# summmeer/session-based-news-recommendation

Measured on AMD Instinct MI355X. Metric: sessions/sec TCAR train on Globo (synthetic globo fold), higher is better.
Workload: dtype bf16 (logits GEMM on split-bf16 planes = 3 MFMAs per product, gradient GEMMs plain bf16; fp32 accumulate, fp32 master state)

## Files before the change

session-based-news-recommendation_amd/csrc/gemm_f32.hip:

```cpp
#include "tcar_common.h"
#include "tcar_bf16_layout.h"
#include <stdlib.h>

typedef __attribute__((ext_vector_type(16))) float f32x16;

constexpr int BK = 32;
constexpr int MAXP = 10;
constexpr int MAXSEG = 3;

struct GemmProb {
  const float* A[MAXSEG];
  const float* B[MAXSEG];
  long lda[MAXSEG], ldb[MAXSEG];
  int K[MAXSEG];
  int nseg;
  float* C;
  long ldc;
  const float* bias;
  int M, N, act, beta;
  int ksplit, kchunk, mode;
  int mt, nt, wg_begin;
  int dact; const float* dact_y; long ld_dact_y; float* colsum;
  __bf16* plane_hi; __bf16* plane_lo; int plane_in32, plane_col0;
  __bf16* pack_hi; __bf16* pack_lo; int pack_in32, pack_c0, pack_c1;
};
struct GroupArgs {
  int nprob;
  int wg0[MAXP];
  GemmProb p[MAXP];
  TcarSignal sig;
};

template <int LAY, int ROWS>
struct TileGeo {
  static constexpr int KC_LD = BK + 4;
  static constexpr int MC_LD = ROWS + 4;
  static constexpr int FLOATS = (LAY == 0) ? ROWS * KC_LD : BK * MC_LD;
  static constexpr int NV = ROWS * BK / 4 / 256;
};

template <int LAY, int ROWS>
__device__ __forceinline__ void load_tile(const float* __restrict__ P, long ld, int r0, int rmax, int k0, int kend,
                                          int tid, float4 (&reg)[TileGeo<LAY, ROWS>::NV]) {
#pragma unroll
  for (int i = 0; i < TileGeo<LAY, ROWS>::NV; ++i) {
    const int f = tid + 256 * i;
    if (LAY == 0) {
      const int row = f >> 3, c4 = f & 7;
      const int gr = r0 + row, gk = k0 + c4 * 4;
      reg[i] = (gr < rmax && gk < kend) ? ld4(P + (long)gr * ld + gk) : zero4();
    } else {
      constexpr int C4 = ROWS / 4;
      const int krow = f / C4, c4 = f - krow * C4;
      const int gk = k0 + krow, gr = r0 + c4 * 4;
      reg[i] = (gk < kend && gr + 3 < rmax) ? ld4(P + (long)gk * ld + gr) : zero4();
    }
  }
}
template <int LAY, int ROWS>
__device__ __forceinline__ void store_tile(float* __restrict__ S, int tid, const float4 (&reg)[TileGeo<LAY, ROWS>::NV]) {
#pragma unroll
  for (int i = 0; i < TileGeo<LAY, ROWS>::NV; ++i) {
    const int f = tid + 256 * i;
    if (LAY == 0) {
      const int row = f >> 3, c4 = f & 7;
      st4(S + row * TileGeo<LAY, ROWS>::KC_LD + c4 * 4, reg[i]);
    } else {
      constexpr int C4 = ROWS / 4;
      const int krow = f / C4, c4 = f - krow * C4;
      st4(S + krow * TileGeo<LAY, ROWS>::MC_LD + c4 * 4, reg[i]);
    }
  }
}
template <int LAY, int ROWS>
__device__ __forceinline__ void read_frag(const float* __restrict__ S, int idx, int c, int h, float (&out)[4]) {
  if (LAY == 0) {
    const float4 v = ld4(S + idx * TileGeo<LAY, ROWS>::KC_LD + c * 8 + 4 * h);
    out[0] = v.x; out[1] = v.y; out[2] = v.z; out[3] = v.w;
  } else {
#pragma unroll
    for (int j = 0; j < 4; ++j) out[j] = S[(c * 8 + 4 * h + j) * TileGeo<LAY, ROWS>::MC_LD + idx];
  }
}

template <int LA, int LB, int TM, int TN>
__global__ __launch_bounds__(256, 2) void gemm_f32_kernel(const GroupArgs ga) {
  extern __shared__ __attribute__((aligned(16))) float smem[];
  constexpr int FM = TM / 64, FN = TN / 64;
  constexpr int A_FL = TileGeo<LA, TM>::FLOATS, B_FL = TileGeo<LB, TN>::FLOATS;
  constexpr int STAGE = A_FL + B_FL;
  const int tid = threadIdx.x;
  const int wave = tid >> 6, lane = tid & 63;
  const int wm = wave >> 1, wn = wave & 1;
  const int li = lane & 31, lh = lane >> 5;

  const int nwg = gridDim.x, bid = blockIdx.x;
  const int xcd = bid & 7, q = nwg >> 3, r = nwg & 7;
  int id = (xcd < r ? xcd * (q + 1) : r * (q + 1) + (xcd - r) * q) + (bid >> 3);
  int pi = 0;
#pragma unroll
  for (int i = 1; i < MAXP; ++i) pi += (id >= ga.wg0[i]) ? 1 : 0;
  const GemmProb& g = ga.p[pi];
  id -= g.wg_begin;
  const int tiles = g.mt * g.nt;
  const int split = id / tiles;
  id -= split * tiles;
  int tm, tn;
  if (g.mt <= g.nt) { tn = id / g.mt; tm = id - tn * g.mt; } else { tm = id / g.nt; tn = id - tm * g.nt; }
  const int m0 = tm * TM, n0 = tn * TN;

  f32x16 acc[FM][FN];
#pragma unroll
  for (int a = 0; a < FM; ++a)
#pragma unroll
    for (int b = 0; b < FN; ++b)
#pragma unroll
      for (int e = 0; e < 16; ++e) acc[a][b][e] = 0.f;

  float4 ra[TileGeo<LA, TM>::NV], rb[TileGeo<LB, TN>::NV];
#pragma unroll 1
  for (int sg = 0; sg < g.nseg; ++sg) {
    const float* __restrict__ Ap = g.A[sg];
    const float* __restrict__ Bp = g.B[sg];
    const long lda = g.lda[sg], ldb = g.ldb[sg];
    const int Kseg = g.K[sg];
    const int ks = split * g.kchunk;
    const int ke = min(Kseg, ks + g.kchunk);
    const int nit = (ke - ks + BK - 1) / BK;
    const int a_rmax = (LA == 0) ? g.M : min((int)lda, (g.M + 3) & ~3);
    const int b_rmax = (LB == 0) ? g.N : min((int)ldb, (g.N + 3) & ~3);
    if (nit > 0) {
      load_tile<LA, TM>(Ap, lda, m0, a_rmax, ks, ke, tid, ra);
      load_tile<LB, TN>(Bp, ldb, n0, b_rmax, ks, ke, tid, rb);
      __syncthreads();
      store_tile<LA, TM>(smem, tid, ra);
      store_tile<LB, TN>(smem + A_FL, tid, rb);
    }
    __syncthreads();
    for (int it = 0; it < nit; ++it) {
      const float* As = smem + (it & 1) * STAGE;
      const float* Bs = As + A_FL;
      const bool more = (it + 1 < nit);
      if (more) {
        load_tile<LA, TM>(Ap, lda, m0, a_rmax, ks + (it + 1) * BK, ke, tid, ra);
        load_tile<LB, TN>(Bp, ldb, n0, b_rmax, ks + (it + 1) * BK, ke, tid, rb);
      }
#pragma unroll
      for (int c = 0; c < BK / 8; ++c) {
        float a[FM][4], b[FN][4];
#pragma unroll
        for (int s = 0; s < FM; ++s) read_frag<LA, TM>(As, wm * (TM / 2) + s * 32 + li, c, lh, a[s]);
#pragma unroll
        for (int s = 0; s < FN; ++s) read_frag<LB, TN>(Bs, wn * (TN / 2) + s * 32 + li, c, lh, b[s]);
#pragma unroll
        for (int j = 0; j < 4; ++j)
#pragma unroll
          for (int s = 0; s < FM; ++s)
#pragma unroll
            for (int t = 0; t < FN; ++t)
              acc[s][t] = __builtin_amdgcn_mfma_f32_32x32x2f32(a[s][j], b[t][j], acc[s][t], 0, 0, 0);
      }
      if (more) {
        float* An = smem + ((it + 1) & 1) * STAGE;
        store_tile<LA, TM>(An, tid, ra);
        store_tile<LB, TN>(An + A_FL, tid, rb);
      }
      __syncthreads();
    }
  }

  float* Cs = g.C + (g.mode == 1 ? (long)split * g.M * g.ldc : 0L);
#pragma unroll
  for (int s = 0; s < FM; ++s)
#pragma unroll
    for (int t = 0; t < FN; ++t) {
      const int col = n0 + wn * (TN / 2) + t * 32 + li;
      if (col >= g.N) continue;
      const float bv = g.bias ? g.bias[col] : 0.f;
#pragma unroll
      for (int e = 0; e < 16; ++e) {
        const int row = m0 + wm * (TM / 2) + s * 32 + (e & 3) + 8 * (e >> 2) + 4 * lh;
        if (row < g.M) {
          float* p = Cs + (long)row * g.ldc + col;
          if (g.mode == 2) {
            atomicAdd(p, acc[s][t][e]);
          } else {
            float v = acc[s][t][e] + bv;
            if (g.act == 1) v = fmaxf(v, 0.f);
            else if (g.act == 2) v = tanhf(v);
            if (g.beta) v += *p;
            *p = v;
          }
        }
      }
    }
}

__global__ __launch_bounds__(256) void splitk_reduce_kernel(const float* __restrict__ slabs, int splitk, int M, int N,
                                                             long ld, float* __restrict__ out) {
  const long n4 = N >> 2;
  const long total = (long)M * n4;
  for (long i = (long)blockIdx.x * blockDim.x + threadIdx.x; i < total; i += (long)gridDim.x * blockDim.x) {
    const long row = i / n4, c = (i - row * n4) * 4;
    float4 s = zero4();
    for (int k = 0; k < splitk; ++k) s = add4(s, ld4(slabs + ((long)k * M + row) * ld + c));
    st4(out + row * ld + c, s);
  }
}

typedef __attribute__((ext_vector_type(8))) __bf16 xbf16x8;
typedef __attribute__((ext_vector_type(4))) __bf16 xbf16x4;
constexpr int X3_MC = 192;
template <int XK> struct X3 {
  static constexpr int KC = 2 * XK + 16;
  static constexpr int PLANE = XK * X3_MC;
  static constexpr int NV = 64 * XK / 4 / 256;
};

typedef float v4f __attribute__((ext_vector_type(4)));
__device__ __forceinline__ v4f gload16_hidden(const float* p) {
  v4f v;
  asm volatile("global_load_dwordx4 %0, %1, off" : "=v"(v) : "v"(p) : "memory");
  return v;
}
template <int N, int NV>
__device__ __forceinline__ void x3_wait(v4f (&a)[NV], v4f (&b)[NV]) {
  static_assert(NV == 2 || NV == 4 || NV == 8, "stage depth 32 / 64 / 128");
  if constexpr (NV == 2)
    asm volatile("s_waitcnt vmcnt(%4)" : "+v"(a[0]), "+v"(a[1]), "+v"(b[0]), "+v"(b[1]) : "n"(N) : "memory");
  else if constexpr (NV == 4)
    asm volatile("s_waitcnt vmcnt(%8)"
                 : "+v"(a[0]), "+v"(a[1]), "+v"(a[2]), "+v"(a[3]), "+v"(b[0]), "+v"(b[1]), "+v"(b[2]), "+v"(b[3])
                 : "n"(N) : "memory");
  else
    asm volatile("s_waitcnt vmcnt(%16)"
                 : "+v"(a[0]), "+v"(a[1]), "+v"(a[2]), "+v"(a[3]), "+v"(a[4]), "+v"(a[5]), "+v"(a[6]), "+v"(a[7]), "+v"(b[0]),
                   "+v"(b[1]), "+v"(b[2]), "+v"(b[3]), "+v"(b[4]), "+v"(b[5]), "+v"(b[6]), "+v"(b[7])
                 : "n"(N) : "memory");
}

template <int LAY, int XK>
__device__ __forceinline__ unsigned x3_load(const float* __restrict__ P, long ld, int r0, int rmax, int k0, int kend, int tid,
                                            v4f (&reg)[X3<XK>::NV]) {
  unsigned mask = 0;
#pragma unroll
  for (int i = 0; i < X3<XK>::NV; ++i) {
    const int f = tid + 256 * i;
    bool ok;
    long off;
    if (LAY == 0) {
      const int row = f / (XK / 4), c4 = f % (XK / 4);
      const int gr = r0 + row, gk = k0 + c4 * 4;
      ok = gr < rmax && gk < kend;
      off = (long)gr * ld + gk;
    } else {
      const int krow = f >> 4, c4 = f & 15;
      const int gk = k0 + krow, gr = r0 + c4 * 4;
      ok = gk < kend && gr + 3 < rmax;
      off = (long)gk * ld + gr;
    }
    reg[i] = gload16_hidden(P + (ok ? off : 0L));
    mask |= ok ? (1u << i) : 0u;
  }
  return mask;
}
template <int LAY, int XK, bool HI = false>
__device__ __forceinline__ void x3_store(char* __restrict__ hi, char* __restrict__ lo, int tid, const v4f (&reg)[X3<XK>::NV],
                                         unsigned mask) {
#pragma unroll
  for (int i = 0; i < X3<XK>::NV; ++i) {
    const int f = tid + 256 * i;
    const bool ok = (mask >> i) & 1u;
    const float v[4] = {ok ? reg[i].x : 0.f, ok ? reg[i].y : 0.f, ok ? reg[i].z : 0.f, ok ? reg[i].w : 0.f};
    xbf16x4 h, l;
#pragma unroll
    for (int j = 0; j < 4; ++j) { h[j] = (__bf16)v[j]; l[j] = HI ? (__bf16)0.f : (__bf16)(v[j] - (float)h[j]); }
    int off;
    if (LAY == 0) { const int row = f / (XK / 4), c4 = f % (XK / 4); off = row * X3<XK>::KC + c4 * 8; }
    else { const int krow = f >> 4, c4 = f & 15; off = krow * X3_MC + c4 * 8; }
    *reinterpret_cast<xbf16x4*>(hi + off) = h;
    if (!HI) *reinterpret_cast<xbf16x4*>(lo + off) = l;
  }
}
template <int LAY, int XK>
__device__ __forceinline__ xbf16x8 x3_frag(const char* __restrict__ S, int base, int s, int lane) {
  if (LAY == 0) {
    return *reinterpret_cast<const xbf16x8*>(S + (base + (lane & 31)) * X3<XK>::KC + s * 32 + (lane >> 5) * 16);
  } else {
    const int g = lane >> 4, i = lane & 15;
    const int mbase = 16 * (g & 1), kbase = 8 * (g >> 1), q = i >> 2, p = i & 3;
    const char* a0 = S + (s * 16 + kbase + q) * X3_MC + (base + mbase + 4 * p) * 2;
    typedef __attribute__((address_space(3))) xbf16x4* lds_p;
    const xbf16x4 lo = __builtin_amdgcn_ds_read_tr16_b64_v4bf16((lds_p)(a0));
    const xbf16x4 hi = __builtin_amdgcn_ds_read_tr16_b64_v4bf16((lds_p)(a0 + 4 * X3_MC));
    return __builtin_shufflevector(lo, hi, 0, 1, 2, 3, 4, 5, 6, 7);
  }
}

template <int LA, int LB, int XK, int XD, bool HI = false>
__global__ __launch_bounds__(256) void gemm_x3_kernel(const GroupArgs ga) {
  constexpr int X3_PLANE = X3<XK>::PLANE, X3_NV = X3<XK>::NV;
  extern __shared__ __attribute__((aligned(16))) float smem_f[];
  char* smem = reinterpret_cast<char*>(smem_f);
  constexpr int T = 64;
  const int tid = threadIdx.x, wave = tid >> 6, lane = tid & 63;
  const int wm = wave >> 1, wn = wave & 1;
  const int nwg = gridDim.x, bid = blockIdx.x;
  const int xcd = bid & 7, q = nwg >> 3, r = nwg & 7;
  int id = (xcd < r ? xcd * (q + 1) : r * (q + 1) + (xcd - r) * q) + (bid >> 3);
  int pi = 0;
#pragma unroll
  for (int i = 1; i < MAXP; ++i) pi += (id >= ga.wg0[i]) ? 1 : 0;
  const GemmProb& g = ga.p[pi];
  id -= g.wg_begin;
  const int tiles = g.mt * g.nt;
  const int split = id / tiles;
  id -= split * tiles;
  int tm, tn;
  if (g.mt <= g.nt) { tn = id / g.mt; tm = id - tn * g.mt; } else { tm = id / g.nt; tn = id - tm * g.nt; }
  const int m0 = tm * T, n0 = tn * T;

  const int ks = split * g.kchunk;
  int cst[MAXSEG + 1];
  cst[0] = 0;
#pragma unroll
  for (int sg = 0; sg < MAXSEG; ++sg) {
    int n = 0;
    if (sg < g.nseg) {
      const int ke = min(g.K[sg], ks + g.kchunk);
      n = ke > ks ? (ke - ks + XK - 1) / XK : 0;
    }
    cst[sg + 1] = cst[sg] + n;
  }
  const int total = cst[MAXSEG];
  const int a_rmax0 = (LA == 0) ? g.M : (g.M + 3) & ~3;
  const int b_rmax0 = (LB == 0) ? g.N : (g.N + 3) & ~3;

  auto stage_seg = [&](int s) { return min((s >= cst[1] ? 1 : 0) + (s >= cst[2] ? 1 : 0), g.nseg - 1); };
  auto load_stage = [&](int s, v4f (&ra)[X3_NV], v4f (&rb)[X3_NV], unsigned& ma, unsigned& mb) {
    const int sg = stage_seg(s);
    const int k0 = ks + (s - cst[sg]) * XK;
    const int ke = min(g.K[sg], ks + g.kchunk);
    const long lda = g.lda[sg], ldb = g.ldb[sg];
    const int a_rmax = (LA == 0) ? a_rmax0 : min((int)lda, a_rmax0);
    const int b_rmax = (LB == 0) ? b_rmax0 : min((int)ldb, b_rmax0);
    ma = x3_load<LA, XK>(g.A[sg], lda, m0, a_rmax, k0, ke, tid, ra);
    mb = x3_load<LB, XK>(g.B[sg], ldb, n0, b_rmax, k0, ke, tid, rb);
  };

  f32x16 acc;
#pragma unroll
  for (int e = 0; e < 16; ++e) acc[e] = 0.f;
  v4f ra[XD][X3_NV], rb[XD][X3_NV];
  unsigned ma[XD], mb[XD];
#pragma unroll
  for (int d = 0; d < XD; ++d) load_stage(d, ra[d], rb[d], ma[d], mb[d]);
#pragma unroll 1
  for (int base = 0; base < total; base += XD) {
#pragma unroll
    for (int d = 0; d < XD; ++d) {
      const int s = base + d;
      __syncthreads();
      x3_wait<(XD - 1) * 2 * X3_NV, X3_NV>(ra[d], rb[d]);
      x3_store<LA, XK, HI>(smem, smem + X3_PLANE, tid, ra[d], ma[d]);
      x3_store<LB, XK, HI>(smem + 2 * X3_PLANE, smem + 3 * X3_PLANE, tid, rb[d], mb[d]);
      __syncthreads();
      load_stage(s + XD, ra[d], rb[d], ma[d], mb[d]);
      const int sg = stage_seg(s);
      const int k0 = ks + (s - cst[sg]) * XK;
      const int left = min(g.K[sg], ks + g.kchunk) - k0;
      const int nsub = s < total ? (min(XK, left + 15) >> 4) : 0;
#pragma unroll 2
      for (int u = 0; u < nsub; ++u) {
        const xbf16x8 ah = x3_frag<LA, XK>(smem, wm * 32, u, lane), bh = x3_frag<LB, XK>(smem + 2 * X3_PLANE, wn * 32, u, lane);
        if constexpr (!HI) {
          const xbf16x8 al = x3_frag<LA, XK>(smem + X3_PLANE, wm * 32, u, lane), bl = x3_frag<LB, XK>(smem + 3 * X3_PLANE, wn * 32, u, lane);
          acc = __builtin_amdgcn_mfma_f32_32x32x16_bf16(al, bh, acc, 0, 0, 0);
          acc = __builtin_amdgcn_mfma_f32_32x32x16_bf16(ah, bl, acc, 0, 0, 0);
        }
        acc = __builtin_amdgcn_mfma_f32_32x32x16_bf16(ah, bh, acc, 0, 0, 0);
      }
    }
  }
  asm volatile("s_waitcnt vmcnt(0)" ::: "memory");
  float* Cs = g.C + (g.mode == 1 ? (long)split * g.M * g.ldc : 0L);
  const bool wt = ga.sig.cnt != nullptr;
  const int col = n0 + wn * 32 + (lane & 31);
  float csum = 0.f;
  if (col < g.N) {
    const float bv = g.bias ? g.bias[col] : 0.f;
    const int gcol = g.plane_col0 + col;
    const bool packed = g.pack_hi && (gcol < g.pack_c0 || gcol >= g.pack_c1);
    const int pcol = gcol < g.pack_c0 ? gcol : gcol - (g.pack_c1 - g.pack_c0);
#pragma unroll
    for (int e = 0; e < 16; ++e) {
      const int row = m0 + wm * 32 + (e & 3) + 8 * (e >> 2) + 4 * (lane >> 5);
      if (row < g.M) {
        float* p = Cs + (long)row * g.ldc + col;
        if (g.mode == 2) {
          atomicAdd(p, acc[e]);
        } else {
          float v = acc[e] + bv;
          if (g.act == 1) v = fmaxf(v, 0.f);
          else if (g.act == 2) v = tanhf(v);
          if (g.dact) {
            const float y = g.dact_y[(long)row * g.ld_dact_y + col];
            v = g.dact == 1 ? (y > 0.f ? v : 0.f) : v * (1.f - y * y);
            csum += v;
          }
          if (g.beta) v += *p;
          if (wt) __hip_atomic_store(p, v, __ATOMIC_RELAXED, __HIP_MEMORY_SCOPE_AGENT);
          else *p = v;
          if (g.plane_hi) {
            const __bf16 h = (__bf16)v, l = (__bf16)(v - (float)h);
            const long o = kb32_off(row, gcol, g.plane_in32);
            g.plane_hi[o] = h;
            g.plane_lo[o] = l;
            if (packed) {
              const long po = kb32_off(row, pcol, g.pack_in32);
              g.pack_hi[po] = h;
              g.pack_lo[po] = l;
            }
          }
        }
      }
    }
  }
  if (g.dact && g.colsum) {
    csum += __shfl_xor(csum, 32);
    if (lane < 32 && col < g.N && csum != 0.f) atomicAdd(g.colsum + col, csum);
  }
  tcar_signal_done(ga.sig);
}

namespace {

template <int LA, int LB, int TM, int TN>
int launch_variant(const GroupArgs& ga, int nwg, hipStream_t st) {
  constexpr size_t lds = 2 * (TileGeo<LA, TM>::FLOATS + TileGeo<LB, TN>::FLOATS) * sizeof(float);
  TCAR_SET_LDS_ONCE((gemm_f32_kernel<LA, LB, TM, TN>), lds);
  TCAR_LAUNCH((gemm_f32_kernel<LA, LB, TM, TN>), dim3(nwg), dim3(256), lds, st, ga);
  TCAR_CHECK_LAUNCH();
  return TCAR_OK;
}

template <int LA, int LB>
int launch_layout(GroupArgs& ga, hipStream_t st) {
  long big = 0;
  for (int i = 0; i < ga.nprob; ++i)
    big += (long)((ga.p[i].M + 127) / 128) * ((ga.p[i].N + 127) / 128) * ga.p[i].ksplit;
  const int T = big >= 192 ? 128 : 64;
  int wg = 0;
  for (int i = 0; i < ga.nprob; ++i) {
    GemmProb& p = ga.p[i];
    p.mt = (p.M + T - 1) / T;
    p.nt = (p.N + T - 1) / T;
    p.wg_begin = wg;
    ga.wg0[i] = wg;
    wg += p.mt * p.nt * p.ksplit;
  }
  for (int i = ga.nprob; i < MAXP; ++i) ga.wg0[i] = 0x7fffffff;
  if (T == 128) return launch_variant<LA, LB, 128, 128>(ga, wg, st);
  return launch_variant<LA, LB, 64, 64>(ga, wg, st);
}

template <int LA, int LB, int XK, int XD, bool HI = false>
int launch_x3_v(GroupArgs& ga, int wg, hipStream_t st, TcarOpt* o) {
  constexpr size_t lds = 4 * X3<XK>::PLANE;
  if (o && o->sig.cnt)
    for (int i = 0; i < ga.nprob; ++i)
      if (ga.p[i].plane_hi || ga.p[i].pack_hi) return TCAR_E_ARG;
  ga.sig = tcar_sig(o);
  TCAR_SET_LDS_ONCE((gemm_x3_kernel<LA, LB, XK, XD, HI>), lds);
  TCAR_LAUNCH((gemm_x3_kernel<LA, LB, XK, XD, HI>), dim3(wg), dim3(256), lds, st, ga);
  TCAR_CHECK_LAUNCH();
  return TCAR_OK;
}

template <int LA, int LB>
int launch_x3(GroupArgs& ga, hipStream_t st, TcarOpt* o) {
  int wg = 0;
  for (int i = 0; i < ga.nprob; ++i) {
    GemmProb& p = ga.p[i];
    p.mt = (p.M + 63) / 64;
    p.nt = (p.N + 63) / 64;
    p.wg_begin = wg;
    ga.wg0[i] = wg;
    wg += p.mt * p.nt * p.ksplit;
  }
  for (int i = ga.nprob; i < MAXP; ++i) ga.wg0[i] = 0x7fffffff;
  int max_stages = 0;
  for (int i = 0; i < ga.nprob; ++i) {
    const GemmProb& p = ga.p[i];
    int n = 0;
    for (int sg = 0; sg < p.nseg; ++sg) n += ((p.K[sg] < p.kchunk ? p.K[sg] : p.kchunk) + 63) / 64;
    max_stages = n > max_stages ? n : max_stages;
  }
  if constexpr (LA == LB)
    if (o && o->hi_only)
      return max_stages <= tcar_fixed::x3_oneshot ? launch_x3_v<LA, LB, 64, 2, true>(ga, wg, st, o) : launch_x3_v<LA, LB, 64, 1, true>(ga, wg, st, o);
  if (max_stages <= tcar_fixed::x3_oneshot) return launch_x3_v<LA, LB, 64, 2>(ga, wg, st, o);
  if constexpr (tcar_fixed::x3_deep != 0)
    if (wg <= 256) return launch_x3_v<LA, LB, 128, 1>(ga, wg, st, o);
  return launch_x3_v<LA, LB, 64, 1>(ga, wg, st, o);
}

int fill_prob(GemmProb& p, int layout, const tcar_gemm_desc_t& d) {
  if (d.M <= 0 || d.N <= 0 || d.nseg < 1 || d.nseg > MAXSEG || !d.C) return TCAR_E_ARG;
  const bool a_kc = (layout != 2), b_kc = (layout == 1);
  p.nseg = d.nseg;
  for (int s = 0; s < d.nseg; ++s) {
    if (!d.A[s] || !d.B[s] || d.K[s] <= 0 || !tcar_aligned16(d.A[s]) || !tcar_aligned16(d.B[s]) || (d.lda[s] & 3) ||
        (d.ldb[s] & 3))
      return TCAR_E_ARG;
    if ((a_kc || b_kc) && (d.K[s] & 3)) return TCAR_E_ARG;
    p.A[s] = d.A[s]; p.B[s] = d.B[s]; p.lda[s] = d.lda[s]; p.ldb[s] = d.ldb[s]; p.K[s] = d.K[s];
  }
  p.C = d.C; p.ldc = d.ldc; p.bias = d.bias; p.M = d.M; p.N = d.N; p.act = d.act; p.beta = d.beta;
  p.dact = d.dact; p.dact_y = d.dact_y; p.ld_dact_y = d.ld_dact_y; p.colsum = d.colsum;
  if (d.dact && (d.dact < 1 || d.dact > 2 || !d.dact_y)) return TCAR_E_ARG;
  p.plane_hi = (__bf16*)d.plane_hi; p.plane_lo = (__bf16*)d.plane_lo; p.plane_in32 = d.plane_inner >> 5; p.plane_col0 = d.plane_col0;
  p.pack_hi = (__bf16*)d.pack_hi; p.pack_lo = (__bf16*)d.pack_lo; p.pack_in32 = d.pack_inner >> 5;
  p.pack_c0 = d.pack_c0; p.pack_c1 = d.pack_c1;
  if (d.plane_hi && (!d.plane_lo || (d.plane_inner & 31) || d.plane_col0 < 0 || d.plane_col0 + d.N > d.plane_inner)) return TCAR_E_ARG;
  if (d.pack_hi && (!d.plane_hi || !d.pack_lo || (d.pack_inner & 31) || d.pack_c0 > d.pack_c1)) return TCAR_E_ARG;
  if ((d.dact || d.plane_hi) && d.splitk > 1) return TCAR_E_ARG;
  int splitk = d.splitk < 1 ? 1 : d.splitk;
  p.mode = splitk > 1 ? (d.atomic ? 2 : 1) : 0;
  if (splitk > 1 && (d.nseg != 1 || d.bias || d.act || d.beta)) return TCAR_E_ARG;
  int kmax = 0;
  for (int s = 0; s < d.nseg; ++s) kmax = d.K[s] > kmax ? d.K[s] : kmax;
  int kchunk = (kmax + splitk - 1) / splitk;
  kchunk = ((kchunk + BK - 1) / BK) * BK;
  p.kchunk = kchunk;
  p.ksplit = (kmax + kchunk - 1) / kchunk;
  if (p.ksplit == 1) p.mode = (splitk > 1 && d.atomic) ? 2 : 0;
  return TCAR_OK;
}

}

extern "C" int tcar_gemm_f32_grouped(int layout, int nprob, const tcar_gemm_desc_t* descs, void* stream) {
  if (nprob <= 0) return TCAR_OK;
  if (layout < 0 || layout > 2 || nprob > MAXP || !descs) return TCAR_E_ARG;
  GroupArgs ga;
  ga.nprob = 0;
  for (int i = 0; i < nprob; ++i) {
    if (descs[i].M <= 0 || descs[i].N <= 0) continue;
    const int rc = fill_prob(ga.p[ga.nprob], layout, descs[i]);
    if (rc) return rc;
    ga.nprob++;
  }
  if (ga.nprob == 0) return TCAR_OK;
  hipStream_t st = (hipStream_t)stream;
  if (layout == 0) return launch_layout<0, 1>(ga, st);
  if (layout == 1) return launch_layout<0, 0>(ga, st);
  return launch_layout<1, 1>(ga, st);
}

extern "C" int tcar_gemm_x3_grouped(int layout, int nprob, const tcar_gemm_desc_t* descs, void* stream) {
  return tcar_gemm_x3_grouped_o(layout, nprob, descs, stream, nullptr);
}
int tcar_gemm_x3_grouped_o(int layout, int nprob, const tcar_gemm_desc_t* descs, void* stream, TcarOpt* o) {
  if (nprob <= 0) return TCAR_OK;
  if (layout < 0 || layout > 2 || nprob > MAXP || !descs) return TCAR_E_ARG;
  GroupArgs ga;
  ga.nprob = 0;
  for (int i = 0; i < nprob; ++i) {
    if (descs[i].M <= 0 || descs[i].N <= 0) continue;
    const int rc = fill_prob(ga.p[ga.nprob], layout, descs[i]);
    if (rc) return rc;
    ga.nprob++;
  }
  if (ga.nprob == 0) return TCAR_OK;
  hipStream_t st = (hipStream_t)stream;
  if (layout == 0) return launch_x3<0, 1>(ga, st, o);
  if (layout == 1) return launch_x3<0, 0>(ga, st, o);
  return launch_x3<1, 1>(ga, st, o);
}

extern "C" int tcar_gemm_f32(int layout, int M, int N, int K, const float* A, int64_t lda, const float* B, int64_t ldb,
                             float* C, int64_t ldc, const float* bias, int act, int beta, int splitk, void* stream) {
  if (M <= 0 || N <= 0 || K <= 0) return TCAR_OK;
  tcar_gemm_desc_t d = {};
  d.nseg = 1;
  d.A[0] = A; d.B[0] = B; d.lda[0] = lda; d.ldb[0] = ldb; d.K[0] = K;
  d.C = C; d.ldc = ldc; d.bias = bias; d.M = M; d.N = N; d.act = act; d.beta = beta; d.splitk = splitk; d.atomic = 0;
  return tcar_gemm_f32_grouped(layout, 1, &d, stream);
}

extern "C" int tcar_gemm_splitk_effective(int K, int splitk) {
  if (splitk < 1) splitk = 1;
  int kchunk = (K + splitk - 1) / splitk;
  kchunk = ((kchunk + BK - 1) / BK) * BK;
  return (K + kchunk - 1) / kchunk;
}

extern "C" int tcar_splitk_reduce(const float* slabs, int splitk, int M, int N, int64_t ld, float* out, void* stream) {
  if (M <= 0 || N <= 0) return TCAR_OK;
  if ((N & 3) || (ld & 3) || !tcar_aligned16(slabs) || !tcar_aligned16(out)) return TCAR_E_ARG;
  long total = (long)M * (N >> 2);
  int blocks = (int)((total + 255) / 256);
  if (blocks > 2048) blocks = 2048;
  TCAR_LAUNCH(splitk_reduce_kernel, dim3(blocks), dim3(256), 0, (hipStream_t)stream, slabs, splitk, M, N, (long)ld, out);
  TCAR_CHECK_LAUNCH();
  return TCAR_OK;
}
```

Baseline: 1.229 million.

## Restructure split-bf16 GEMM main loop with pointer cursors and software-pipelined LDS reads

Replaces per-stage index recomputation with incremental pointer cursors that walk K, tracking segment switches via a running k-left counter. Adds an unmasked fast path for full interior tiles and derives the bf16 hi residual with bit operations. The inner MFMA loop is fully unrolled and issues LDS fragment reads two sub-steps ahead with explicit lgkmcnt waits, which should overlap LDS latency with MFMA. It also sets launch bounds to 3 blocks per CU, which adds register pressure and spill risk.

Result: faster. 1.242 million, median of 6 (+1.1%).

```diff
diff --git a/session-based-news-recommendation_amd/csrc/gemm_f32.hip b/session-based-news-recommendation_amd/csrc/gemm_f32.hip
--- a/session-based-news-recommendation_amd/csrc/gemm_f32.hip
+++ b/session-based-news-recommendation_amd/csrc/gemm_f32.hip
@@ -1,6 +1,7 @@
 #include "tcar_common.h"
 #include "tcar_bf16_layout.h"
 #include <stdlib.h>
+#include <utility>
 
 typedef __attribute__((ext_vector_type(16))) float f32x16;
 
@@ -218,6 +219,8 @@
 };
 
 typedef float v4f __attribute__((ext_vector_type(4)));
+typedef unsigned x3_u32x2 __attribute__((ext_vector_type(2)));
+constexpr int X3_AHEAD = 2;
 __device__ __forceinline__ v4f gload16_hidden(const float* p) {
   v4f v;
   asm volatile("global_load_dwordx4 %0, %1, off" : "=v"(v) : "v"(p) : "memory");
@@ -240,41 +243,70 @@
 }
 
 template <int LAY, int XK>
-__device__ __forceinline__ unsigned x3_load(const float* __restrict__ P, long ld, int r0, int rmax, int k0, int kend, int tid,
-                                            v4f (&reg)[X3<XK>::NV]) {
-  unsigned mask = 0;
+struct X3Cursor {
+  static constexpr int NV = X3<XK>::NV;
+  static constexpr int NP = LAY == 0 ? NV : 1;
+  const char* p[NP];
+  const char* base;
+  long step, row16;
+  unsigned rows;
+  int kc;
+
+  __device__ __forceinline__ void seek(const float* __restrict__ P, long ld, int r0, int rmax, int k0, int tid) {
+    base = reinterpret_cast<const char*>(P);
+    rows = 0;
+    if (LAY == 0) {
+      constexpr int C4 = XK / 4, RS = 256 / C4;
+      const int row = tid / C4, c4 = tid % C4;
+      kc = c4 * 4;
+      step = (long)XK * 4;
+#pragma unroll
+      for (int i = 0; i < NV; ++i) {
+        const int gr = r0 + row + RS * i;
+        const bool ok = gr < rmax;
+        rows |= ok ? (1u << i) : 0u;
+        p[i] = base + ((long)(ok ? gr : 0) * ld + k0 + kc) * 4;
+      }
+    } else {
+      const int krow = tid >> 4, gr = r0 + (tid & 15) * 4;
+      const bool ok = gr + 3 < rmax;
+      kc = krow;
+      step = (long)XK * ld * 4;
+      rows = ok ? (1u << NV) - 1u : 0u;
+      row16 = 16 * ld * 4;
+      p[0] = base + ((long)(k0 + krow) * ld + (ok ? gr : 0)) * 4;
+    }
+  }
+  __device__ __forceinline__ unsigned load(int kleft, v4f (&reg)[NV]) {
+    unsigned mask = 0;
+#pragma unroll
+    for (int i = 0; i < NV; ++i) {
+      const bool kok = (LAY == 0 ? kc : kc + 16 * i) < kleft;
+      const char* a = LAY == 0 ? p[i] : p[0] + i * row16;
+      reg[i] = gload16_hidden(reinterpret_cast<const float*>(kok ? a : base));
+      mask |= kok ? (1u << i) : 0u;
+    }
+#pragma unroll
+    for (int i = 0; i < NP; ++i) p[i] += step;
+    return mask & rows;
+  }
+};
+template <int LAY, int XK, bool HI, bool MASKED>
+__device__ __forceinline__ void x3_store(char* __restrict__ hi, char* __restrict__ lo, int tid, const v4f (&reg)[X3<XK>::NV],
+                                         unsigned mask) {
 #pragma unroll
   for (int i = 0; i < X3<XK>::NV; ++i) {
     const int f = tid + 256 * i;
-    bool ok;
-    long off;
-    if (LAY == 0) {
-      const int row = f / (XK / 4), c4 = f % (XK / 4);
-      const int gr = r0 + row, gk = k0 + c4 * 4;
-      ok = gr < rmax && gk < kend;
-      off = (long)gr * ld + gk;
-    } else {
-      const int krow = f >> 4, c4 = f & 15;
-      const int gk = k0 + krow, gr = r0 + c4 * 4;
-      ok = gk < kend && gr + 3 < rmax;
-      off = (long)gk * ld + gr;
-    }
-    reg[i] = gload16_hidden(P + (ok ? off : 0L));
-    mask |= ok ? (1u << i) : 0u;
-  }
-  return mask;
-}
-template <int LAY, int XK, bool HI = false>
-__device__ __forceinline__ void x3_store(char* __restrict__ hi, char* __restrict__ lo, int tid, const v4f (&reg)[X3<XK>::NV],
-                                         unsigned mask) {
-#pragma unroll
-  for (int i = 0; i < X3<XK>::NV; ++i) {
-    const int f = tid + 256 * i;
-    const bool ok = (mask >> i) & 1u;
+    const bool ok = !MASKED || ((mask >> i) & 1u);
     const float v[4] = {ok ? reg[i].x : 0.f, ok ? reg[i].y : 0.f, ok ? reg[i].z : 0.f, ok ? reg[i].w : 0.f};
     xbf16x4 h, l;
 #pragma unroll
-    for (int j = 0; j < 4; ++j) { h[j] = (__bf16)v[j]; l[j] = HI ? (__bf16)0.f : (__bf16)(v[j] - (float)h[j]); }
+    for (int j = 0; j < 4; ++j) h[j] = (__bf16)v[j];
+    const x3_u32x2 hb = __builtin_bit_cast(x3_u32x2, h);
+    const float hf[4] = {__uint_as_float(hb.x << 16), __uint_as_float(hb.x & 0xffff0000u), __uint_as_float(hb.y << 16),
+                         __uint_as_float(hb.y & 0xffff0000u)};
+#pragma unroll
+    for (int j = 0; j < 4; ++j) l[j] = HI ? (__bf16)0.f : (__bf16)(v[j] - hf[j]);
     int off;
     if (LAY == 0) { const int row = f / (XK / 4), c4 = f % (XK / 4); off = row * X3<XK>::KC + c4 * 8; }
     else { const int krow = f >> 4, c4 = f & 15; off = krow * X3_MC + c4 * 8; }
@@ -283,23 +315,43 @@
   }
 }
 template <int LAY, int XK>
-__device__ __forceinline__ xbf16x8 x3_frag(const char* __restrict__ S, int base, int s, int lane) {
-  if (LAY == 0) {
-    return *reinterpret_cast<const xbf16x8*>(S + (base + (lane & 31)) * X3<XK>::KC + s * 32 + (lane >> 5) * 16);
-  } else {
-    const int g = lane >> 4, i = lane & 15;
-    const int mbase = 16 * (g & 1), kbase = 8 * (g >> 1), q = i >> 2, p = i & 3;
-    const char* a0 = S + (s * 16 + kbase + q) * X3_MC + (base + mbase + 4 * p) * 2;
-    typedef __attribute__((address_space(3))) xbf16x4* lds_p;
-    const xbf16x4 lo = __builtin_amdgcn_ds_read_tr16_b64_v4bf16((lds_p)(a0));
-    const xbf16x4 hi = __builtin_amdgcn_ds_read_tr16_b64_v4bf16((lds_p)(a0 + 4 * X3_MC));
-    return __builtin_shufflevector(lo, hi, 0, 1, 2, 3, 4, 5, 6, 7);
-  }
-}
+__device__ __forceinline__ unsigned x3_frag_addr(const char* S, int base, int lane) {
+  typedef __attribute__((address_space(3))) const char* lds_c;
+  const unsigned s0 = (unsigned)(unsigned long)(lds_c)S;
+  if (LAY == 0) return s0 + (base + (lane & 31)) * X3<XK>::KC + (lane >> 5) * 16;
+  const int g = lane >> 4, i = lane & 15;
+  const int mbase = 16 * (g & 1), kbase = 8 * (g >> 1), q = i >> 2, p = i & 3;
+  return s0 + (kbase + q) * X3_MC + (base + mbase + 4 * p) * 2;
+}
+template <int LAY> constexpr int X3_STEP = LAY == 0 ? 32 : 16 * X3_MC;
+template <int LAY> struct X3Frag;
+template <> struct X3Frag<0> {
+  static constexpr int READS = 1;
+  xbf16x8 v;
+  template <int OFF> __device__ __forceinline__ void issue(unsigned a) {
+    asm volatile("ds_read_b128 %0, %1 offset:%2" : "=v"(v) : "v"(a), "n"(OFF) : "memory");
+  }
+  template <int N> __device__ __forceinline__ void land() { asm volatile("s_waitcnt lgkmcnt(%1)" : "+v"(v) : "n"(N) : "memory"); }
+  __device__ __forceinline__ xbf16x8 get() const { return v; }
+};
+template <> struct X3Frag<1> {
+  static constexpr int READS = 2;
+  xbf16x4 lo, hi;
+  template <int OFF> __device__ __forceinline__ void issue(unsigned a) {
+    asm volatile("ds_read_b64_tr_b16 %0, %1 offset:%2" : "=v"(lo) : "v"(a), "n"(OFF) : "memory");
+    asm volatile("ds_read_b64_tr_b16 %0, %1 offset:%2" : "=v"(hi) : "v"(a), "n"(OFF + 4 * X3_MC) : "memory");
+  }
+  template <int N> __device__ __forceinline__ void land() {
+    asm volatile("s_waitcnt lgkmcnt(%2)" : "+v"(lo), "+v"(hi) : "n"(N) : "memory");
+  }
+  __device__ __forceinline__ xbf16x8 get() const { return __builtin_shufflevector(lo, hi, 0, 1, 2, 3, 4, 5, 6, 7); }
+};
+template <int... U, class F>
+__device__ __forceinline__ void x3_unrolled(std::integer_sequence<int, U...>, F&& f) { (f(std::integral_constant<int, U>{}), ...); }
 
 template <int LA, int LB, int XK, int XD, bool HI = false>
-__global__ __launch_bounds__(256) void gemm_x3_kernel(const GroupArgs ga) {
-  constexpr int X3_PLANE = X3<XK>::PLANE, X3_NV = X3<XK>::NV;
+__global__ __launch_bounds__(256, 3) void gemm_x3_kernel(const GroupArgs ga) {
+  constexpr int X3_PLANE = X3<XK>::PLANE, X3_NV = X3<XK>::NV, NS = XK / 16;
   extern __shared__ __attribute__((aligned(16))) float smem_f[];
   char* smem = reinterpret_cast<char*>(smem_f);
   constexpr int T = 64;
@@ -313,72 +365,109 @@
   for (int i = 1; i < MAXP; ++i) pi += (id >= ga.wg0[i]) ? 1 : 0;
   const GemmProb& g = ga.p[pi];
   id -= g.wg_begin;
-  const int tiles = g.mt * g.nt;
-  const int split = id / tiles;
-  id -= split * tiles;
+  int split = 0;
+  if (g.ksplit > 1) {
+    const int tiles = g.mt * g.nt;
+    split = id / tiles;
+    id -= split * tiles;
+  }
   int tm, tn;
   if (g.mt <= g.nt) { tn = id / g.mt; tm = id - tn * g.mt; } else { tm = id / g.nt; tn = id - tm * g.nt; }
   const int m0 = tm * T, n0 = tn * T;
 
-  const int ks = split * g.kchunk;
-  int cst[MAXSEG + 1];
-  cst[0] = 0;
+  const int ks = split * g.kchunk, nseg = g.nseg;
+  const float *sA[MAXSEG], *sB[MAXSEG];
+  long sla[MAXSEG], slb[MAXSEG];
+  int sk[MAXSEG], total = 0;
 #pragma unroll
   for (int sg = 0; sg < MAXSEG; ++sg) {
-    int n = 0;
-    if (sg < g.nseg) {
-      const int ke = min(g.K[sg], ks + g.kchunk);
-      n = ke > ks ? (ke - ks + XK - 1) / XK : 0;
-    }
-    cst[sg + 1] = cst[sg] + n;
-  }
-  const int total = cst[MAXSEG];
+    sA[sg] = g.A[sg]; sB[sg] = g.B[sg]; sla[sg] = g.lda[sg]; slb[sg] = g.ldb[sg];
+    sk[sg] = sg < nseg ? max(min(g.K[sg], ks + g.kchunk) - ks, 0) : 0;
+    total += (sk[sg] + XK - 1) / XK;
+  }
   const int a_rmax0 = (LA == 0) ? g.M : (g.M + 3) & ~3;
   const int b_rmax0 = (LB == 0) ? g.N : (g.N + 3) & ~3;
 
-  auto stage_seg = [&](int s) { return min((s >= cst[1] ? 1 : 0) + (s >= cst[2] ? 1 : 0), g.nseg - 1); };
-  auto load_stage = [&](int s, v4f (&ra)[X3_NV], v4f (&rb)[X3_NV], unsigned& ma, unsigned& mb) {
-    const int sg = stage_seg(s);
-    const int k0 = ks + (s - cst[sg]) * XK;
-    const int ke = min(g.K[sg], ks + g.kchunk);
-    const long lda = g.lda[sg], ldb = g.ldb[sg];
+  X3Cursor<LA, XK> ca;
+  X3Cursor<LB, XK> cb;
+  int cseg = 0, kleft;
+  bool inner;
+  auto seek = [&](const float* A, const float* B, long lda, long ldb, int k) {
     const int a_rmax = (LA == 0) ? a_rmax0 : min((int)lda, a_rmax0);
     const int b_rmax = (LB == 0) ? b_rmax0 : min((int)ldb, b_rmax0);
-    ma = x3_load<LA, XK>(g.A[sg], lda, m0, a_rmax, k0, ke, tid, ra);
-    mb = x3_load<LB, XK>(g.B[sg], ldb, n0, b_rmax, k0, ke, tid, rb);
+    ca.seek(A, lda, m0, a_rmax, ks, tid);
+    cb.seek(B, ldb, n0, b_rmax, ks, tid);
+    inner = m0 + T <= a_rmax && n0 + T <= b_rmax;
+    kleft = k;
   };
-
+  seek(sA[0], sB[0], sla[0], slb[0], sk[0]);
+  auto load_stage = [&](v4f (&ra)[X3_NV], v4f (&rb)[X3_NV], unsigned& msk, int& kl, bool& full) {
+    kl = kleft;
+    full = inner && kleft >= XK;
+    msk = ca.load(kleft, ra);
+    msk |= cb.load(kleft, rb) << X3_NV;
+    kleft = __builtin_amdgcn_readfirstlane(max(kleft - XK, 0));
+    if (kleft == 0 && cseg + 1 < nseg) {
+      ++cseg;
+      const bool one = cseg == 1;
+      seek(one ? sA[1] : sA[2], one ? sB[1] : sB[2], one ? sla[1] : sla[2], one ? slb[1] : slb[2], one ? sk[1] : sk[2]);
+    }
+  };
+
+  v4f ra[XD][X3_NV], rb[XD][X3_NV];
+  unsigned msk[XD];
+  int kl[XD];
+  bool full[XD];
+#pragma unroll
+  for (int d = 0; d < XD; ++d) load_stage(ra[d], rb[d], msk[d], kl[d], full[d]);
   f32x16 acc;
 #pragma unroll
   for (int e = 0; e < 16; ++e) acc[e] = 0.f;
-  v4f ra[XD][X3_NV], rb[XD][X3_NV];
-  unsigned ma[XD], mb[XD];
-#pragma unroll
-  for (int d = 0; d < XD; ++d) load_stage(d, ra[d], rb[d], ma[d], mb[d]);
+  char* const Ah = smem, *const Al = smem + X3_PLANE, *const Bh = smem + 2 * X3_PLANE, *const Bl = smem + 3 * X3_PLANE;
+  const unsigned fa = x3_frag_addr<LA, XK>(Ah, wm * 32, lane), fb = x3_frag_addr<LB, XK>(Bh, wn * 32, lane);
 #pragma unroll 1
   for (int base = 0; base < total; base += XD) {
 #pragma unroll
     for (int d = 0; d < XD; ++d) {
-      const int s = base + d;
       __syncthreads();
       x3_wait<(XD - 1) * 2 * X3_NV, X3_NV>(ra[d], rb[d]);
-      x3_store<LA, XK, HI>(smem, smem + X3_PLANE, tid, ra[d], ma[d]);
-      x3_store<LB, XK, HI>(smem + 2 * X3_PLANE, smem + 3 * X3_PLANE, tid, rb[d], mb[d]);
+      if (full[d]) {
+        x3_store<LA, XK, HI, false>(Ah, Al, tid, ra[d], 0u);
+        x3_store<LB, XK, HI, false>(Bh, Bl, tid, rb[d], 0u);
+      } else {
+        x3_store<LA, XK, HI, true>(Ah, Al, tid, ra[d], msk[d]);
+        x3_store<LB, XK, HI, true>(Bh, Bl, tid, rb[d], msk[d] >> X3_NV);
+      }
       __syncthreads();
-      load_stage(s + XD, ra[d], rb[d], ma[d], mb[d]);
-      const int sg = stage_seg(s);
-      const int k0 = ks + (s - cst[sg]) * XK;
-      const int left = min(g.K[sg], ks + g.kchunk) - k0;
-      const int nsub = s < total ? (min(XK, left + 15) >> 4) : 0;
-#pragma unroll 2
-      for (int u = 0; u < nsub; ++u) {
-        const xbf16x8 ah = x3_frag<LA, XK>(smem, wm * 32, u, lane), bh = x3_frag<LB, XK>(smem + 2 * X3_PLANE, wn * 32, u, lane);
-        if constexpr (!HI) {
-          const xbf16x8 al = x3_frag<LA, XK>(smem + X3_PLANE, wm * 32, u, lane), bl = x3_frag<LB, XK>(smem + 3 * X3_PLANE, wn * 32, u, lane);
-          acc = __builtin_amdgcn_mfma_f32_32x32x16_bf16(al, bh, acc, 0, 0, 0);
-          acc = __builtin_amdgcn_mfma_f32_32x32x16_bf16(ah, bl, acc, 0, 0, 0);
-        }
-        acc = __builtin_amdgcn_mfma_f32_32x32x16_bf16(ah, bh, acc, 0, 0, 0);
+      const int nsub = (min(XK, max(kl[d], 0)) + 15) >> 4;
+      load_stage(ra[d], rb[d], msk[d], kl[d], full[d]);
+      if (nsub > 0) {
+        X3Frag<LA> ah[NS], al[NS];
+        X3Frag<LB> bh[NS], bl[NS];
+        constexpr int R = (HI ? 1 : 2) * (X3Frag<LA>::READS + X3Frag<LB>::READS);
+        auto issue = [&](auto U) {
+          constexpr int u = decltype(U)::value, oa = u * X3_STEP<LA>, ob = u * X3_STEP<LB>;
+          if constexpr (!HI) { al[u].template issue<X3_PLANE + oa>(fa); bh[u].template issue<ob>(fb); }
+          ah[u].template issue<oa>(fa);
+          if constexpr (!HI) bl[u].template issue<X3_PLANE + ob>(fb);
+          else bh[u].template issue<ob>(fb);
+        };
+        x3_unrolled(std::make_integer_sequence<int, X3_AHEAD>{}, issue);
+        x3_unrolled(std::make_integer_sequence<int, NS>{}, [&](auto U) {
+          constexpr int u = decltype(U)::value;
+          constexpr int Y = R * (NS - 1 - u < X3_AHEAD - 1 ? NS - 1 - u : X3_AHEAD - 1);
+          if constexpr (!HI) { al[u].template land<Y>(); bl[u].template land<Y>(); }
+          ah[u].template land<Y>();
+          bh[u].template land<Y>();
+          if (u == 0 || u < nsub) {
+            if constexpr (!HI) {
+              acc = __builtin_amdgcn_mfma_f32_32x32x16_bf16(al[u].get(), bh[u].get(), acc, 0, 0, 0);
+              acc = __builtin_amdgcn_mfma_f32_32x32x16_bf16(ah[u].get(), bl[u].get(), acc, 0, 0, 0);
+            }
+            acc = __builtin_amdgcn_mfma_f32_32x32x16_bf16(ah[u].get(), bh[u].get(), acc, 0, 0, 0);
+          }
+          if constexpr (u + X3_AHEAD < NS) issue(std::integral_constant<int, u + X3_AHEAD>{});
+        });
       }
     }
   }
```
